# google-research/nerf-from-image

Hardware: NVIDIA H100
Metric: rays_per_sec_128x128_64+64spp (higher is better)
Workload: dtype f32

## Files before the change

nerf_from_image_b200/csrc/nfi_forward_pipe.cuh:

```cuda
#pragma once
#include <type_traits>

#include "nfi_forward.cuh"
#include "nfi_forward_tc.cuh"

namespace nfi {

#ifndef NFI_WAIT_NS
#define NFI_WAIT_NS 0
#endif
#define NFI_STEP_WAIT(bar, par) tc::mbar_wait_backoff<NFI_WAIT_NS>(bar, par)

__device__ __forceinline__ void mbar_arrive(uint64_t* bar) {
  asm volatile("mbarrier.arrive.shared::cta.b64 _, [%0];" ::"r"(tc::smem_u32(bar)) : "memory");
}

__device__ __forceinline__ float ld_relaxed(const float* p) {
  float v;
  asm volatile("ld.relaxed.cta.global.f32 %0, [%1];" : "=f"(v) : "l"(p) : "memory");
  return v;
}

__device__ __forceinline__ bool elect_one() {
  uint32_t pred;
  asm volatile(
      "{\n.reg .pred p;\nelect.sync _|p, 0xffffffff;\nselp.u32 %0, 1, 0, p;\n}\n"
      : "=r"(pred));
  return pred != 0;
}

struct TileCoord {
  int b, tile_x, tile_y;
};

__device__ __forceinline__ TileCoord tile_coord(int tile, int tiles_x, int tiles_y) {
  TileCoord c;
  const int per_img = tiles_x * tiles_y;
  c.b = tile / per_img;
  const int r = tile % per_img;
  const int bx = (tiles_x + 1) / 2;
  const int blk = r / 4, in = r % 4;
  int tx = 2 * (blk % bx) + (in & 1), ty = 2 * (blk / bx) + (in >> 1);
  if ((tiles_x & 1) || (tiles_y & 1)) {
    tx = r % tiles_x;
    ty = r / tiles_x;
  }
  c.tile_x = tx;
  c.tile_y = ty;
  return c;
}

constexpr int kPipeSlots = 3;
constexpr int kPipeStageBytes = 32768;
constexpr int kFwdStageBytes = 16384;
constexpr int kD2Ld = 20;
constexpr int kD2SlotBytes = kThreads * kD2Ld * 4;

__host__ __device__ inline size_t pipe_scratch_floats(int S, int nes) {
  return tc_scratch_floats_per_group(S) + (size_t)S * kThreads * nes;
}

constexpr int kViewTileBytes = kThreads * NFI_VIEW_FEATURES * 4;

template <int P, bool VD = false>
struct PipeCfg {
  static constexpr int kThreadsTotal = 256 + 128 * P;
  static constexpr int kStages = P + 1;
  static constexpr int kSmA = VD ? 41984 : 25600;
  static constexpr int kSmD2 = kSmA + kStages * kFwdStageBytes;
  static constexpr int kSmView = kSmD2 + kPipeSlots * kD2SlotBytes;
  static constexpr int kSmPal = kSmView + (VD ? kViewTileBytes : 0);
  static constexpr int kSmFrac = kSmPal + 48 * 4;
  static constexpr int kSmBars = kSmFrac + 128 * 4;
  static constexpr int kNumBars = 2 * kStages + 2 * kPipeSlots + 3;
  static constexpr int kSmBytes = kSmBars + kNumBars * 8;
  static constexpr int kActRegs = 136;
  static constexpr int kShadeRegs = 80;
  static constexpr int kProducerRegs = 88;
};

constexpr float kLog2e = 1.4426950408889634f;
constexpr float kLn2 = 0.6931471805599453f;
constexpr float kPadLogit = -1e30f;

__device__ __forceinline__ void decoder_layer2(const float (&d)[32], uint64_t w2_hi, uint64_t w2_lo,
                                               const float* __restrict__ b1, float* d2, int warp,
                                               int lane) {
  uint32_t hi[8][4], lo[8][4];
  tc::softplus_frag<true>(d, b1, lane & 3, hi, lo);
  float o[8];
#pragma unroll
  for (int i = 0; i < 8; ++i) o[i] = 0.f;
  tc::wgmma_fence();
  tc::layer2_mb(o, hi, lo, w2_hi, w2_lo);
  tc::wgmma_commit();
  tc::wgmma_wait<0>();
  tc::reg_fence(o);
  tc::store_frag_rows(o, d2, kD2Ld, warp, lane);
}

template <typename F>
__device__ __forceinline__ void decoder_step(uint64_t dsc_a, uint64_t w1_hi, uint64_t w1_lo,
                                             uint64_t w2_hi, uint64_t w2_lo,
                                             const float* __restrict__ b1, float* d2, int warp,
                                             int lane, F&& on_stage_read) {
#pragma unroll 1
  for (int mb = 0; mb < 2; ++mb) {
    float d[32];
#pragma unroll
    for (int i = 0; i < 32; ++i) d[i] = 0.f;
    tc::wgmma_fence();
    tc::layer1_mb(d, dsc_a + mb * (8192 >> 4), dsc_a + ((16384 + mb * 8192) >> 4), w1_hi, w1_lo);
    tc::wgmma_commit();
    tc::wgmma_wait<0>();
    tc::reg_fence(d);
    if (mb == 1) on_stage_read();
    decoder_layer2(d, w2_hi, w2_lo, b1, d2 + 64 * mb * kD2Ld, warp, lane);
  }
}

template <typename F>
__device__ __forceinline__ void decoder_step_fp32(const unsigned char* stage, uint64_t w1_hi,
                                                  uint64_t w1_lo, uint64_t w2_hi, uint64_t w2_lo,
                                                  const float* __restrict__ b1, float* d2, int warp,
                                                  int lane, F&& on_stage_read) {
  float fa[4][4], fb[4][4];
  tc::load_afrag_sw128(fa, stage, 0, warp, lane);
  tc::load_afrag_sw128(fb, stage, 64, warp, lane);
  on_stage_read();
#pragma unroll 1
  for (int mb = 0; mb < 2; ++mb) {
    uint32_t a_hi[4][4], a_lo[4][4];
#pragma unroll
    for (int kb = 0; kb < 4; ++kb)
#pragma unroll
      for (int s = 0; s < 4; ++s) tc::put_split(a_hi, a_lo, kb, s, fa[kb][s]);
    float d[32];
#pragma unroll
    for (int i = 0; i < 32; ++i) d[i] = 0.f;
    tc::wgmma_fence();
    tc::layer1_mb_rs(d, a_hi, a_lo, w1_hi, w1_lo);
    tc::wgmma_commit();
    tc::wgmma_wait<0>();
    tc::reg_fence(d);
    decoder_layer2(d, w2_hi, w2_lo, b1, d2 + 64 * mb * kD2Ld, warp, lane);
#pragma unroll
    for (int kb = 0; kb < 4; ++kb)
#pragma unroll
      for (int s = 0; s < 4; ++s) fa[kb][s] = fb[kb][s];
  }
}

__device__ __forceinline__ void fill_view_tile(const nfi_render_params& p, const TileCoord& tcd,
                                               const float* __restrict__ b2f, float4* vt, int wig,
                                               int lane) {
  const int g = lane >> 2, t = lane & 3;
#pragma unroll
  for (int mb = 0; mb < 2; ++mb) {
    const float* src[2];
#pragma unroll
    for (int h = 0; h < 2; ++h) {
      const int row = 64 * mb + 16 * wig + g + 8 * h;
      int px, py;
      tile_pixel(tcd.tile_x, tcd.tile_y, row >> 5, row & 31, px, py);
      px = min(px, p.width - 1);
      py = min(py, p.height - 1);
      const size_t ray = ((size_t)tcd.b * p.height + py) * p.width + px;
      src[h] = p.view_features + ray * NFI_VIEW_FEATURES + 2 * t;
    }
#pragma unroll
    for (int j = 0; j < NFI_VIEW_FEATURES / 8; ++j) {
      const float2 a = __ldg(reinterpret_cast<const float2*>(src[0] + 8 * j));
      const float2 c = __ldg(reinterpret_cast<const float2*>(src[1] + 8 * j));
      const float2 bb = *reinterpret_cast<const float2*>(b2f + 8 * j + 2 * t);
      vt[(mb * 4 + j) * kThreads] = make_float4(a.x + bb.x, a.y + bb.y, c.x + bb.x, c.y + bb.y);
    }
  }
}

__device__ __forceinline__ uint32_t decoder_layers23_vd(const float (&d)[32], uint64_t w2_hi,
                                                        uint64_t w2_lo, uint64_t w3_hi,
                                                        uint64_t w3_lo, const float* __restrict__ b1,
                                                        const float4* vt, float* d2, int warp,
                                                        int lane) {
  uint32_t hi[8][4], lo[8][4];
  tc::softplus_frag<true>(d, b1, lane & 3, hi, lo);
  float o[20];
#pragma unroll
  for (int i = 0; i < 20; ++i) o[i] = 0.f;
  tc::wgmma_fence();
  tc::layer2_vd_mb(o, hi, lo, w2_hi, w2_lo);
  tc::wgmma_commit();
  tc::wgmma_wait<0>();
  tc::reg_fence(o);
  uint32_t yhi[4][4], ylo[4][4];
  uint32_t neg = 0;
#pragma unroll
  for (int j = 0; j < 4; ++j) {
    const float4 v = vt[j * kThreads];
    const float ve[4] = {v.x, v.y, v.z, v.w};
#pragma unroll
    for (int e = 0; e < 4; ++e) {
      const float z = o[4 * j + e] + ve[e];
      tc::put_split(yhi, ylo, j, tc::afrag_slot(e), z > 0.f ? z : z * 0.2f);
      neg |= (z > 0.f ? 0u : 1u) << (4 * j + e);
    }
  }
  float q[8];
#pragma unroll
  for (int i = 0; i < 8; ++i) q[i] = 0.f;
  tc::wgmma_fence();
  tc::layer3_vd_mb(q, yhi, ylo, w3_hi, w3_lo);
  tc::wgmma_commit();
  tc::wgmma_wait<0>();
  tc::reg_fence(q);
  if ((lane & 3) == 0) {
    q[0] = o[16];
    q[2] = o[18];
  }
  tc::store_frag_rows(q, d2, kD2Ld, warp, lane);
  return neg;
}

template <typename F>
__device__ __forceinline__ uint32_t decoder_step_vd(const unsigned char* stage, uint64_t w1_hi,
                                                uint64_t w1_lo, uint64_t w2_hi, uint64_t w2_lo,
                                                uint64_t w3_hi, uint64_t w3_lo,
// ... 70 lines not shown
#pragma unroll
    for (int a = 0; a < NA; ++a) {
      const float e = tc::ex2_approx(out[1 + a] - m);
      if (probs != nullptr) probs[a] = e;
      s += e;
      r = fmaf(e, pv[3 * a + 0], r);
      g = fmaf(e, pv[3 * a + 1], g);
      b = fmaf(e, pv[3 * a + 2], b);
    }
    const float inv = __fdividef(1.f, s);
    cr = r * inv;
    cg = g * inv;
    cb = b * inv;
    if (probs != nullptr) {
#pragma unroll
      for (int a = 0; a < NA; ++a) probs[a] *= inv;
    }
  } else {
    cr = sigmoid_fast(out[1]) * 2.004f - 1.002f;
    cg = sigmoid_fast(out[2]) * 2.004f - 1.002f;
    cb = sigmoid_fast(out[3]) * 2.004f - 1.002f;
  }
}

template <int N>
struct LaneVec {
  float v[N];
};
template <int N>
__device__ __forceinline__ LaneVec<N> shift_down1(const LaneVec<N>& x, float pad, int lane) {
  LaneVec<N> y;
#pragma unroll
  for (int i = 0; i < N; ++i) {
    const float a = __shfl_down_sync(kFull, x.v[i], 1);
    const float nxt0 = (i + 1 < N) ? __shfl_sync(kFull, x.v[(i + 1 < N) ? i + 1 : i], 0) : pad;
    y.v[i] = (lane == 31) ? nxt0 : a;
  }
  return y;
}
template <int N>
__device__ __forceinline__ float pick(const LaneVec<N>& x, int idx) {
  float r = __shfl_sync(kFull, x.v[0], idx & 31);
#pragma unroll
  for (int i = 1; i < N; ++i) {
    const float t = __shfl_sync(kFull, x.v[i], idx & 31);
    r = ((idx >> 5) == i) ? t : r;
  }
  return r;
}
template <int N>
__device__ __forceinline__ void bitonic_sort(LaneVec<N>& x, int lane) {
#pragma unroll
  for (int k = 2; k <= 32 * N; k <<= 1) {
#pragma unroll
    for (int j = k >> 1; j > 0; j >>= 1) {
      if (j >= 32) {
        const int dj = j >> 5;
#pragma unroll
        for (int i = 0; i < N; ++i) {
          if ((i & dj) == 0) {
            const int ip = i | dj;
            const bool asc = (k >= 32 * N) ? true : (((32 * i) & k) == 0);
            const float lo = fminf(x.v[i], x.v[ip]), hi = fmaxf(x.v[i], x.v[ip]);
            x.v[i] = asc ? lo : hi;
            x.v[ip] = asc ? hi : lo;
          }
        }
      } else {
        const bool lower = (lane & j) == 0;
#pragma unroll
        for (int i = 0; i < N; ++i) {
          const float o = __shfl_xor_sync(kFull, x.v[i], j);
          const bool asc = (k >= 32 * N) ? true : (k < 32 ? ((lane & k) == 0) : (((32 * i) & k) == 0));
          x.v[i] = (lower == asc) ? fminf(x.v[i], o) : fmaxf(x.v[i], o);
        }
      }
    }
  }
}

template <int N>
__device__ __forceinline__ LaneVec<N> resample_ray(const LaneVec<N>& w, const LaneVec<N>& t,
                                                   LaneVec<N> u, bool sorted, int S, int lane) {
  const float inf = __int_as_float(0x7f800000);
  const LaneVec<N> w1 = shift_down1<N>(w, 0.f, lane);
  const LaneVec<N> w2 = shift_down1<N>(w1, 0.f, lane);
  LaneVec<N> q;
  float sum = 0.f;
#pragma unroll
  for (int i = 0; i < N; ++i) {
    float pm = ((fmaxf(w.v[i], w1.v[i]) + fmaxf(w1.v[i], w2.v[i])) * 0.5f + 0.01f) + 1e-5f;
    if (32 * i + lane >= S - 2) pm = 0.f;
    q.v[i] = pm;
    sum += pm;
  }
#pragma unroll
  for (int o = 16; o > 0; o >>= 1) sum += __shfl_xor_sync(kFull, sum, o);
#pragma unroll
  for (int i = 0; i < N; ++i) q.v[i] = q.v[i] / sum;
#pragma unroll
  for (int o = 1; o < 32; o <<= 1) {
#pragma unroll
    for (int i = 0; i < N; ++i) {
      const float y = __shfl_up_sync(kFull, q.v[i], o);
      if (lane >= o) q.v[i] += y;
    }
  }
#pragma unroll
  for (int i = 1; i < N; ++i) q.v[i] += __shfl_sync(kFull, q.v[i - 1], 31);
  LaneVec<N> c;
#pragma unroll
  for (int i = 0; i < N; ++i) {
    const float up = __shfl_up_sync(kFull, q.v[i], 1);
    const float prev31 = (i > 0) ? __shfl_sync(kFull, q.v[(i > 0) ? i - 1 : 0], 31) : 0.f;
    c.v[i] = (lane == 0) ? prev31 : up;
    if (32 * i + lane > S - 2) c.v[i] = inf;
  }
  const LaneVec<N> t1 = shift_down1<N>(t, 0.f, lane);
  LaneVec<N> bn;
#pragma unroll
  for (int i = 0; i < N; ++i) bn.v[i] = 0.5f * (t1.v[i] + t.v[i]);
  if (!sorted) bitonic_sort<N>(u, lane);
  LaneVec<N> z;
#pragma unroll
  for (int h = 0; h < N; ++h) {
    const float uu = u.v[h];
    int pos = 0;
#pragma unroll
    for (int s = 16 * N; s > 0; s >>= 1) {
      const float val = pick<N>(c, pos + s - 1);
      if (val <= uu) pos += s;
    }
    const int below = max(pos - 1, 0), above = min(pos, S - 2);
    const float c0 = pick<N>(c, below), c1 = pick<N>(c, above);
    const float b0 = pick<N>(bn, below), b1 = pick<N>(bn, above);
    float den = c1 - c0;
    if (den < 1e-5f) den = 1.f;
    z.v[h] = b0 + (uu - c0) / den * (b1 - b0);
  }
  return z;
}

struct ResampleArgs {
  const float* sc_w;
  float* sc_zf;
  float* z_fine;
  const float* noise_t;
  const float* noise_u;
  const float* frac;
  int S, wig;
  bool explicit_noise;
};
template <int N>
__device__ __forceinline__ void resample_rows_impl(const ResampleArgs& a, int first, int count,
                                                   float tnear, float tfar, size_t ray, bool valid,
                                                   int lane) {
  const int S = a.S;
  if (count <= 0) return;
  struct In {
    LaneVec<N> w, n, u;
    size_t rayj;
  };
  auto load = [&](int j, In& in) {
    in.rayj = ((size_t)__shfl_sync(kFull, (unsigned)(ray >> 32), j) << 32) |
              (size_t)__shfl_sync(kFull, (unsigned)ray, j);
    const int col = 32 * a.wig + j;
#pragma unroll
    for (int i = 0; i < N; ++i) {
      const int e = 32 * i + lane;
      in.w.v[i] = (e < S) ? ldcg(a.sc_w + e * kThreads + col) : 0.f;
      in.n.v[i] = 0.f;
      if (a.explicit_noise) {
        in.n.v[i] = (e < S) ? a.noise_t[in.rayj * S + e] : 0.f;
        in.u.v[i] = (e < S) ? a.noise_u[in.rayj * S + e] : 2.f;
      } else {
        in.u.v[i] = (e < S) ? linspace01(e, S) : 2.f;
      }
    }
  };
  In cur, nxt;
  load(first, cur);
#pragma unroll 1
  for (int j = first; j < first + count; ++j) {
    load(j + 1 < first + count ? j + 1 : j, nxt);
    const float nearj = __shfl_sync(kFull, tnear, j), farj = __shfl_sync(kFull, tfar, j);
    const bool validj = __shfl_sync(kFull, (int)valid, j) != 0;
    const int col = 32 * a.wig + j;
    const float spanj = farj - nearj;
    LaneVec<N> t;
#pragma unroll
    for (int i = 0; i < N; ++i)
      t.v[i] = lerp_torch(nearj, farj, a.frac[32 * i + lane]) + cur.n.v[i] * (spanj / (float)S);
    const LaneVec<N> z = resample_ray<N>(cur.w, t, cur.u, !a.explicit_noise, S, lane);
#pragma unroll
    for (int i = 0; i < N; ++i) {
      const int e = 32 * i + lane;
      if (e < S) a.sc_zf[e * kThreads + col] = z.v[i];
      if (a.z_fine != nullptr && validj && e < S) a.z_fine[cur.rayj * S + e] = z.v[i];
    }
    cur = nxt;
  }
}
template <int NOUT_PAD, int EXTRA, bool FINE, int P, bool DBG, int NSLOT = 2, bool VD = false>
__global__ void __launch_bounds__(PipeCfg<P>::kThreadsTotal, 1)
render_forward_pipe(const nfi_render_params p, const unsigned char* __restrict__ wimg,
                    float* __restrict__ scratch) {
  using Cfg = PipeCfg<P, VD>;
  static_assert(!(VD && DBG), "the phase timers are not instantiated for the view-conditioned kernel");
  constexpr int kImgBytes = VD ? kVdBytes : kWiBytes;
  constexpr int kImgB1 = VD ? kVdB1 : kWiB1, kImgB2 = VD ? kVdHead : kWiB2;
  constexpr int NA_ = NOUT_PAD - 1;
  constexpr int NE = (EXTRA == 1) ? 3 : (EXTRA == 2 ? NA_ : 0);
  constexpr int NES = (EXTRA == 2) ? NA_ : 0;
  extern __shared__ __align__(1024) unsigned char smem_raw[];
  unsigned char* base = smem_raw;
  const int tid = threadIdx.x, lane = tid & 31;
  const int hw_wg = __shfl_sync(kFull, tid >> 7, 0);
  const int wg = (hw_wg < P) ? hw_wg + 3 : (P + 1 - hw_wg);
  const int gt = tid & 127;
  const int wig = __shfl_sync(kFull, gt >> 5, 0);
  const int S = p.num_samples;

  uint64_t* bars = reinterpret_cast<uint64_t*>(base + Cfg::kSmBars);
  constexpr int NS = Cfg::kStages;
  uint64_t* full = bars;
  uint64_t* a_free = full + NS;
  uint64_t* d2_full = a_free + NS;
  uint64_t* slot_free = d2_full + kPipeSlots;
  uint64_t* cw_ready = slot_free + kPipeSlots;
  uint64_t* zf_ready = cw_ready + 1;
  uint64_t* wbar = zf_ready + 1;
  float* d2s = reinterpret_cast<float*>(base + Cfg::kSmD2);
  const float* b1s = reinterpret_cast<const float*>(base + kImgB1);
  const float* b2s = reinterpret_cast<const float*>(base + kImgB2);
  float* pal = reinterpret_cast<float*>(base + Cfg::kSmPal);
  float* frac = reinterpret_cast<float*>(base + Cfg::kSmFrac);
  if (tid < 128) frac[tid] = (float)tid / (float)S;

  if (tid == 0) {
    if (tc::smem_u32(base) & 1023u) __trap();
    for (int i = 0; i < NS; ++i) {
      tc::mbar_init(&full[i], kWarps);
      tc::mbar_init(&a_free[i], kWarps);
    }
    for (int i = 0; i < kPipeSlots; ++i) {
      tc::mbar_init(&d2_full[i], kWarps);
      tc::mbar_init(&slot_free[i], kWarps);
    }
    tc::mbar_init(cw_ready, kWarps);
    tc::mbar_init(zf_ready, (2 + P) * kWarps);
    tc::mbar_init(wbar, 1);
    tc::fence_mbar_init();
  }
  __syncthreads();
  if (tid == 0) {
    tc::mbar_expect_tx(wbar, kImgBytes);
    tc::tma_bulk_g2s(base, wimg, kImgBytes, wbar);
  }
  tc::mbar_wait(wbar, 0);

  const int tiles_x = (p.width + kTileW - 1) / kTileW;
  const int tiles_y = (p.height + kTileH - 1) / kTileH;
  const int n_tiles = tiles_x * tiles_y * p.batch;
  const int my_tiles =
      ((int)blockIdx.x < n_tiles) ? (n_tiles - 1 - (int)blockIdx.x) / (int)gridDim.x + 1 : 0;
  const uint32_t total_steps = (uint32_t)my_tiles * (uint32_t)S * (FINE ? 2u : 1u);
  const int R = p.plane_res;
  const float inv_range = 1.f / p.scene_range;
  const bool explicit_noise = (p.noise_mode == NFI_NOISE_EXPLICIT);
  const bool dbg_skip_gather = (p.mlp_mode & 0x100) != 0;
  const bool dbg_skip_consumer = (p.mlp_mode & 0x200) != 0;
  const bool dbg_window = (p.mlp_mode & 0x800) != 0;
  const bool dbg_time = DBG && (p.mlp_mode & 0x1000) && p.normals != nullptr && blockIdx.x == 0 &&
                        lane == 0 && (wg <= 3) && wg != 2 && wig == 0;
  long long tacc[DBG ? 10 : 1];
  long long tprev = 0;
  if (DBG)
    for (int i = 0; i < 10; ++i) tacc[i] = 0;
#define NFI_T(i)                         \
  if (DBG && dbg_time) {                 \
    const long long now__ = clock64();   \
    tacc[i] += now__ - tprev;            \
    tprev = now__;                       \
  }
  float* slab = scratch + (size_t)blockIdx.x * pipe_scratch_floats(S, NES);
  float4* sc_srgb = reinterpret_cast<float4*>(slab);
  float* sc_t = slab + (size_t)4 * S * kThreads;
  float* sc_w = sc_t + (size_t)S * kThreads;
  float* sc_zf = sc_w + (size_t)S * kThreads;
  float* sc_e = sc_zf + (size_t)S * kThreads;

  constexpr int kRsParts = 2 + P;
  auto rs_first = [](int part) {
    constexpr int base_rows = 32 / kRsParts, rem = 32 % kRsParts;
    return part * base_rows + min(max(part - 2, 0), rem);
  };
  auto resample_rows = [&](int part, float tnear, float tfar, size_t ray, bool valid) {
    const int first = rs_first(part), count = rs_first(part + 1) - first;
    ResampleArgs ra;
    ra.sc_w = sc_w;
    ra.sc_zf = sc_zf;
    ra.z_fine = p.z_fine;
    ra.noise_t = p.noise_t;
    ra.noise_u = p.noise_u;
    ra.frac = frac;
    ra.S = S;
    ra.wig = wig;
    ra.explicit_noise = explicit_noise;
    resample_rows_impl<NSLOT>(ra, first, count, tnear, tfar, ray, valid, lane);
  };

  if (wg >= 3) {
    asm volatile("setmaxnreg.dec.sync.aligned.u32 %0;" ::"n"(Cfg::kProducerRegs));
    const int set = wg - 3;
    uint32_t n = 0;
    uint32_t tile_it = 0;
    for (int tile = blockIdx.x; tile < n_tiles; tile += gridDim.x, ++tile_it) {
      const TileCoord tcd = tile_coord(tile, tiles_x, tiles_y);
      const int b = tcd.b;
      int px, py;
      tile_pixel(tcd.tile_x, tcd.tile_y, wig, lane, px, py);
      const bool valid = (px < p.width) && (py < p.height);
      px = min(px, p.width - 1);
      py = min(py, p.height - 1);
      const size_t ray = ((size_t)b * p.height + py) * p.width + px;
      Ray r;
      setup_ray(p, b, py, px, r);
      const float span = r.tfar - r.tnear;
      const uint32_t plane_bytes = (uint32_t)R * (uint32_t)R * 128u;
      const unsigned char* planes_b =
          reinterpret_cast<const unsigned char*>(p.planes) + (size_t)b * 3 * plane_bytes;
      for (int pass = 0; pass < (FINE ? 2 : 1); ++pass) {
        if (pass == 1) {
          tc::mbar_wait(cw_ready, tile_it & 1);
          resample_rows(2 + set, r.tnear, r.tfar, ray, valid);
          __threadfence_block();
          __syncwarp();
          if (lane == 0) mbar_arrive(zf_ready);
          tc::mbar_wait(zf_ready, tile_it & 1);
        }
        int s = (int)(((uint32_t)set + (uint32_t)P - (n % P)) % P);
        auto fetch = [&](int ss) -> float {
          if (ss >= S) return 0.f;
          if (pass == 0) return explicit_noise ? p.noise_t[ray * S + ss] : 0.f;
          return ld_relaxed(sc_zf + ss * kThreads + gt);
        };
        float nxt = fetch(s);
        for (; s < S; s += P) {
          const uint32_t st = (n + (uint32_t)s) % NS, u = (n + (uint32_t)s) / NS;
          unsigned char* const stage = base + Cfg::kSmA + st * kFwdStageBytes;
          const float cur = nxt;
          nxt = fetch(s + P);
          if (DBG && dbg_time) tprev = clock64();
          NFI_STEP_WAIT(&a_free[st], (u & 1) ^ 1);
          NFI_T(0)
          float t;
          if (pass == 0)
            t = lerp_torch(r.tnear, r.tfar, frac[s]) + cur * (span / (float)S);
          else
            t = cur;
          const float x0 = (r.ox + r.dx * t) * inv_range, x1 = (r.oy + r.dy * t) * inv_range,
                      x2 = (r.oz + r.dz * t) * inv_range;
          ByteTaps tp;
          byte_taps(x0, x1, R, 0u, tp.o[0], tp.fx[0], tp.fy[0]);
          byte_taps(x0, x2, R, plane_bytes >> 4, tp.o[1], tp.fx[1], tp.fy[1]);
          byte_taps(x1, x2, R, plane_bytes >> 3, tp.o[2], tp.fx[2], tp.fy[2]);
          NFI_T(1)
          if (dbg_window) {
            tp.o[0] &= 0x7FFu;
            tp.o[1] &= 0x7FFu;
            tp.o[2] &= 0x7FFu;
          }
          if (!dbg_skip_gather)
            gather_to_tiles_lean<TileStore::kFp32>(planes_b, R, tp, stage, nullptr, 32 * wig, lane);
          NFI_T(2)
          __syncwarp();
          if (lane == 0) mbar_arrive(&full[st]);
          NFI_T(3)
          if (DBG && dbg_time) tacc[9] += 1;
        }
        n += (uint32_t)S;
      }
    }
    if (DBG && dbg_time)
      for (int i = 0; i < 10; ++i) p.normals[i] = (float)tacc[i];
  } else if (wg == 0) {
    asm volatile("setmaxnreg.inc.sync.aligned.u32 %0;" ::"n"(Cfg::kActRegs));
    const uint32_t base_s = tc::smem_u32(base);
    const uint64_t dsc_w1_hi = tc::gmma_desc_sw128(base_s + kWiW1Hi);
    const uint64_t dsc_w1_lo = tc::gmma_desc_sw128(base_s + kWiW1Lo);
    const uint64_t dsc_w2_hi = tc::gmma_desc_sw128(base_s + (VD ? kVdW2Hi : kWiW2Hi));
    const uint64_t dsc_w2_lo = tc::gmma_desc_sw128(base_s + (VD ? kVdW2Lo : kWiW2Lo));
    const float4* vt = reinterpret_cast<const float4*>(base + Cfg::kSmView) + gt;
    uint32_t st = 0, u = 0, sl = 0, v = 0;
    auto activate = [&]() {
      if (DBG && dbg_time && tprev == 0) tprev = clock64();
      NFI_T(2)
      NFI_STEP_WAIT(&full[st], u & 1);
      NFI_STEP_WAIT(&slot_free[sl], (v & 1) ^ 1);
      NFI_T(0)
      float* d2 = d2s + sl * (kThreads * kD2Ld);
      if constexpr (VD) {
        decoder_step_vd(base + Cfg::kSmA + st * kFwdStageBytes, dsc_w1_hi, dsc_w1_lo, dsc_w2_hi,
                        dsc_w2_lo, tc::gmma_desc_sw128(base_s + kVdW3Hi),
                        tc::gmma_desc_sw128(base_s + kVdW3Lo), b1s, vt, d2, wig, lane, [&]() {
                          __syncwarp();
                          if (lane == 0) mbar_arrive(&a_free[st]);
                        });
      } else if (!dbg_skip_consumer) {
        decoder_step_fp32(base + Cfg::kSmA + st * kFwdStageBytes, dsc_w1_hi, dsc_w1_lo, dsc_w2_hi,
                          dsc_w2_lo, b1s, d2, wig, lane, [&]() {
                            __syncwarp();
                            if (lane == 0) mbar_arrive(&a_free[st]);
                          });
      } else {
        __syncwarp();
        if (lane == 0) mbar_arrive(&a_free[st]);
      }
      __syncwarp();
      if (lane == 0) mbar_arrive(&d2_full[sl]);
      if (++st == NS) { st = 0; ++u; }
      if (++sl == kPipeSlots) { sl = 0; ++v; }
      NFI_T(1)
      if (DBG && dbg_time) tacc[9] += 1;
    };
    uint32_t tile_it = 0;
    for (int tile = blockIdx.x; tile < n_tiles; tile += gridDim.x, ++tile_it) {
      if constexpr (VD)
        fill_view_tile(p, tile_coord(tile, tiles_x, tiles_y),
                       reinterpret_cast<const float*>(base + kVdB2f),
                       reinterpret_cast<float4*>(base + Cfg::kSmView) + gt, wig, lane);
      for (int s = 0; s < S; ++s) activate();
      if (FINE) {
        const TileCoord tcd = tile_coord(tile, tiles_x, tiles_y);
        int px, py;
        tile_pixel(tcd.tile_x, tcd.tile_y, wig, lane, px, py);
        const bool valid = (px < p.width) && (py < p.height);
        px = min(px, p.width - 1);
        py = min(py, p.height - 1);
        const size_t ray = ((size_t)tcd.b * p.height + py) * p.width + px;
        Ray r;
        setup_ray(p, tcd.b, py, px, r);
        tc::mbar_wait(cw_ready, tile_it & 1);
        NFI_T(3)
        resample_rows(1, r.tnear, r.tfar, ray, valid);
        __threadfence_block();
        __syncwarp();
        if (lane == 0) mbar_arrive(zf_ready);
        NFI_T(4)
        for (int s = 0; s < S; ++s) activate();
      }
    }
    if (DBG && dbg_time)
      for (int i = 0; i < 10; ++i) p.normals[16 + i] = (float)tacc[i];
  } else {
    asm volatile("setmaxnreg.dec.sync.aligned.u32 %0;" ::"n"(Cfg::kShadeRegs));
    uint32_t sl = 0, v = 0;
    FieldConst fc;
    fc.A = p.n_attention;
    fc.use_sdf = p.use_sdf;
    fc.inv_beta = p.use_sdf ? 1.f / p.beta[0] : 0.f;
    fc.inv_alpha = p.use_sdf ? 1.f / p.alpha[0] : 0.f;

    uint32_t tile_it = 0;
    for (int tile = blockIdx.x; tile < n_tiles; tile += gridDim.x, ++tile_it) {
      const TileCoord tcd = tile_coord(tile, tiles_x, tiles_y);
      const int b = tcd.b;
      int px, py;
      tile_pixel(tcd.tile_x, tcd.tile_y, wig, lane, px, py);
      const bool valid = (px < p.width) && (py < p.height);
      px = min(px, p.width - 1);
      py = min(py, p.height - 1);
      const size_t ray = ((size_t)b * p.height + py) * p.width + px;
      Ray r;
      setup_ray(p, b, py, px, r);
      const float span = r.tfar - r.tnear;

      tc::bar_sync(1, kThreads);
      if (gt < 48)
        pal[gt] = (p.n_attention > 0 && gt < p.n_attention * 3)
                      ? p.palette[(size_t)b * p.n_attention * 3 + gt]
                      : 0.f;
      tc::bar_sync(1, kThreads);
      Compositor<NE, true> comp;
      comp.init();

      auto shade = [&](float t, float& sigma, float& cr, float& cg, float& cb, float* ex) {
        const float* d2 = d2s + sl * (kThreads * kD2Ld) + gt * kD2Ld;
        if (DBG && dbg_time && tprev == 0) tprev = clock64();
        NFI_T(2)
        NFI_STEP_WAIT(&d2_full[sl], v & 1);
        NFI_T(0)
        float o16[16];
#pragma unroll
        for (int o4 = 0; o4 < 4; ++o4) {
          const float4 x = *reinterpret_cast<const float4*>(d2 + 4 * o4);
          o16[4 * o4] = x.x;
          o16[4 * o4 + 1] = x.y;
          o16[4 * o4 + 2] = x.z;
          o16[4 * o4 + 3] = x.w;
        }
        __syncwarp();
        if (lane == 0) mbar_arrive(&slot_free[sl]);
        if (++sl == kPipeSlots) { sl = 0; ++v; }
        const float wx = r.ox + r.dx * t, wy = r.oy + r.dy * t, wz = r.oz + r.dz * t;
        const float x0 = wx * inv_range, x1 = wy * inv_range, x2 = wz * inv_range;
        const float keep =
            (fabsf(x0) > 1.f || fabsf(x1) > 1.f || fabsf(x2) > 1.f) ? 0.f : 1.f;
        float out[NOUT_PAD];
#pragma unroll
        for (int o4 = 0; o4 < NOUT_PAD / 4; ++o4) {
          const float4 bb = *reinterpret_cast<const float4*>(b2s + 4 * o4);
          out[4 * o4] = o16[4 * o4] + bb.x;
          out[4 * o4 + 1] = o16[4 * o4 + 1] + bb.y;
          out[4 * o4 + 2] = o16[4 * o4 + 2] + bb.z;
          out[4 * o4 + 3] = o16[4 * o4 + 3] + bb.w;
        }
        if (dbg_skip_consumer) {
          sigma = out[0];
          cr = cg = cb = out[1];
        } else {
          field_head_fast<NOUT_PAD>(out, fc, pal, keep, sigma, cr, cg, cb,
                                    EXTRA == 2 ? ex : nullptr);
        }
        if (EXTRA == 1) {
          ex[0] = wx;
          ex[1] = wy;
          ex[2] = wz;
        }
        NFI_T(1)
        if (DBG && dbg_time) tacc[9] += 1;
      };

      {
        float wT = 1.f, prev_t = 0.f, prev_s = 0.f;
        const float4* nz4 = reinterpret_cast<const float4*>(p.noise_t + ray * S);
        const float4 zero4 = make_float4(0.f, 0.f, 0.f, 0.f);
        float4 nzc = explicit_noise ? nz4[0] : zero4;
        float4 nzn = (explicit_noise && S > 4) ? nz4[1] : zero4;
        const float jit = span / (float)S;
        for (int s = 0; s < S; ++s) {
          const int sq = s & 3;
          const float nz = sq == 0 ? nzc.x : (sq == 1 ? nzc.y : (sq == 2 ? nzc.z : nzc.w));
          const float t = lerp_torch(r.tnear, r.tfar, frac[s]) + nz * jit;
          if (sq == 3) {
            nzc = nzn;
            nzn = (explicit_noise && s + 5 < S) ? nz4[(s + 5) >> 2] : zero4;
          }
          float sigma, cr, cg, cb;
          float ex[NE > 0 ? NE : 1];
          shade(t, sigma, cr, cg, cb, ex);
          if (FINE) {
            sc_srgb[s * kThreads + gt] = make_float4(sigma, cr, cg, cb);
            sc_t[s * kThreads + gt] = t;
#pragma unroll
            for (int a = 0; a < NES; ++a) sc_e[((size_t)s * NES + a) * kThreads + gt] = ex[a];
            if (s > 0) {
              const float delta = (t - prev_t) * r.dn;
              const float a = 1.f - __expf(-prev_s * delta);
              sc_w[(s - 1) * kThreads + gt] = a * wT;
              wT = wT * ((1.f - a) + 1e-10f);
            }
            prev_t = t;
            prev_s = sigma;
          } else {
            comp.push(t, sigma, cr, cg, cb, ex, r.dn);
          }
          NFI_T(3)
        }
      }

      if (FINE) {
        sc_w[(S - 1) * kThreads + gt] = 0.f;
        __threadfence_block();
        __syncwarp();
        if (lane == 0) mbar_arrive(cw_ready);
        tc::mbar_wait(cw_ready, tile_it & 1);
        NFI_T(4)
        resample_rows(0, r.tnear, r.tfar, ray, valid);
        __threadfence_block();
        __syncwarp();
        if (lane == 0) mbar_arrive(zf_ready);
        tc::mbar_wait(zf_ready, tile_it & 1);
        NFI_T(5)

        int c = 0;
        float ct0 = ldcg(sc_t + gt), ct1 = ldcg(sc_t + kThreads + gt);
        float4 cq0 = __ldcg(sc_srgb + gt), cq1 = __ldcg(sc_srgb + kThreads + gt);
        auto take_coarse = [&]() {
          float ce[NE > 0 ? NE : 1];
          if (EXTRA == 1) {
            ce[0] = r.ox + r.dx * ct0;
            ce[1] = r.oy + r.dy * ct0;
            ce[2] = r.oz + r.dz * ct0;
          }
#pragma unroll
          for (int a = 0; a < NES; ++a) ce[a] = ldcg(sc_e + ((size_t)c * NES + a) * kThreads + gt);
          comp.push(ct0, cq0.x, cq0.y, cq0.z, cq0.w, ce, r.dn);
          ++c;
          ct0 = ct1;
          cq0 = cq1;
          if (c + 1 < S) {
            ct1 = ldcg(sc_t + (c + 1) * kThreads + gt);
            cq1 = __ldcg(sc_srgb + (c + 1) * kThreads + gt);
          }
        };
        float z0 = ldcg(sc_zf + gt);
        float z1 = (S > 1) ? ldcg(sc_zf + kThreads + gt) : 0.f;
        for (int k = 0; k < S; ++k) {
          const float z = z0;
          z0 = z1;
          z1 = (k + 2 < S) ? ldcg(sc_zf + (k + 2) * kThreads + gt) : 0.f;
          float sigma, cr, cg, cb;
          float ex[NE > 0 ? NE : 1];
          shade(z, sigma, cr, cg, cb, ex);
          while (c < S && ct0 <= z) take_coarse();
          comp.push(z, sigma, cr, cg, cb, ex, r.dn);
          NFI_T(3)
        }
        while (c < S) take_coarse();
        NFI_T(6)
      }

      if (valid) {
        float bg = 0.f;
        if (p.white_background) bg = 1.f - comp.am;
        p.rgb[ray * 3 + 0] = comp.ar + bg;
        p.rgb[ray * 3 + 1] = comp.ag + bg;
        p.rgb[ray * 3 + 2] = comp.ab + bg;
        p.depth[ray] = comp.ad;
        p.mask[ray] = comp.am;
        for (int q = 0; q < p.n_peers; ++q) {
          float* pr = p.peer_rgb[q] + ray * 3;
          pr[0] = comp.ar + bg;
          pr[1] = comp.ag + bg;
          pr[2] = comp.ab + bg;
          p.peer_depth[q][ray] = comp.ad;
          p.peer_mask[q][ray] = comp.am;
        }
        if (EXTRA == 1 && p.extra != nullptr)
          for (int a = 0; a < 3; ++a) p.extra[ray * 3 + a] = comp.ae[a];
        if (EXTRA == 2 && p.extra != nullptr)
          for (int a = 0; a < NE; ++a)
            if (a < p.n_attention) p.extra[ray * p.n_attention + a] = comp.ae[a];
      }
    }
    if (DBG && dbg_time)
      for (int i = 0; i < 10; ++i) p.normals[32 + i] = (float)tacc[i];
  }
#undef NFI_T
  __syncthreads();
  if (p.n_peers > 0 && p.peer_done != nullptr && tid == 0) {
    __threadfence_system();
    const unsigned done = atomicAdd(p.peer_done, 1u);
    if (done == gridDim.x - 1) {
      __threadfence();
      *p.peer_done = 0u;
      for (int q = 0; q < p.n_peers; ++q)
        asm volatile("st.release.sys.global.u32 [%0], %1;" ::"l"(p.peer_signal[q]), "r"(p.peer_epoch)
                     : "memory");
      const long long t0 = clock64();
      for (int q = 0; q < p.n_peers; ++q) {
        const uint32_t* flag = p.peer_signal_self + p.peer_rank[q];
        uint32_t v;
        do {
          asm volatile("ld.acquire.sys.global.u32 %0, [%1];" : "=r"(v) : "l"(flag) : "memory");
          if ((int)(v - p.peer_epoch) >= 0) break;
          __nanosleep(200);
          if (clock64() - t0 > 60000000000LL) __trap();
        } while (true);
      }
    }
  }
}

}
```

Before: 36.05 million.

## Interleave coarse pass of next tile with fine pass using double-buffered scratch

Reorders the per-block pass sequence so the coarse pass of tile i+1 runs before the fine pass of tile i, with scratch slabs, palettes and cw/zf barriers double-buffered by tile parity. In the non-VD fine kernel, resampling moves entirely to the producer warpgroups, which interleave resample rows opportunistically whenever the coarse weights are ready and the next stage is not yet free. This is meant to hide the resampling bubble and the full-CTA sync between coarse and fine passes. It costs twice the global scratch, extra barrier bookkeeping, and more complex control flow in the producers.

```diff
diff --git a/nerf_from_image_b200/csrc/nfi_forward_pipe.cuh b/nerf_from_image_b200/csrc/nfi_forward_pipe.cuh
--- a/nerf_from_image_b200/csrc/nfi_forward_pipe.cuh
+++ b/nerf_from_image_b200/csrc/nfi_forward_pipe.cuh
@@ -13,6 +13,17 @@
 
 __device__ __forceinline__ void mbar_arrive(uint64_t* bar) {
   asm volatile("mbarrier.arrive.shared::cta.b64 _, [%0];" ::"r"(tc::smem_u32(bar)) : "memory");
+}
+
+__device__ __forceinline__ bool mbar_test(uint64_t* bar, uint32_t parity) {
+  uint32_t ok;
+  asm volatile(
+      "{\n.reg .pred p;\nmbarrier.test_wait.parity.shared::cta.b64 p, [%1], %2;\n"
+      "selp.u32 %0, 1, 0, p;\n}\n"
+      : "=r"(ok)
+      : "r"(tc::smem_u32(bar)), "r"(parity)
+      : "memory");
+  return ok != 0;
 }
 
 __device__ __forceinline__ float ld_relaxed(const float* p) {
@@ -56,8 +67,11 @@
 constexpr int kD2Ld = 20;
 constexpr int kD2SlotBytes = kThreads * kD2Ld * 4;
 
+__host__ __device__ inline size_t pipe_tile_scratch_floats(int S, int nes) {
+  return tc_scratch_floats_per_group(S) + (size_t)S * kThreads * nes;
+}
 __host__ __device__ inline size_t pipe_scratch_floats(int S, int nes) {
-  return tc_scratch_floats_per_group(S) + (size_t)S * kThreads * nes;
+  return 2 * pipe_tile_scratch_floats(S, nes);
 }
 
 constexpr int kViewTileBytes = kThreads * NFI_VIEW_FEATURES * 4;
@@ -70,9 +84,9 @@
   static constexpr int kSmD2 = kSmA + kStages * kFwdStageBytes;
   static constexpr int kSmView = kSmD2 + kPipeSlots * kD2SlotBytes;
   static constexpr int kSmPal = kSmView + (VD ? kViewTileBytes : 0);
-  static constexpr int kSmFrac = kSmPal + 48 * 4;
+  static constexpr int kSmFrac = kSmPal + 2 * 48 * 4;
   static constexpr int kSmBars = kSmFrac + 128 * 4;
-  static constexpr int kNumBars = 2 * kStages + 2 * kPipeSlots + 3;
+  static constexpr int kNumBars = 2 * kStages + 2 * kPipeSlots + 5;
   static constexpr int kSmBytes = kSmBars + kNumBars * 8;
   static constexpr int kActRegs = 136;
   static constexpr int kShadeRegs = 80;
@@ -449,54 +463,76 @@
   bool explicit_noise;
 };
 template <int N>
+struct ResampleIn {
+  LaneVec<N> w, n, u;
+  size_t rayj;
+};
+template <int N>
+__device__ __forceinline__ void resample_load(const ResampleArgs& a, int j, size_t ray, int lane,
+                                              ResampleIn<N>& in) {
+  const int S = a.S;
+  in.rayj = ((size_t)__shfl_sync(kFull, (unsigned)(ray >> 32), j) << 32) |
+            (size_t)__shfl_sync(kFull, (unsigned)ray, j);
+  const int col = 32 * a.wig + j;
+#pragma unroll
+  for (int i = 0; i < N; ++i) {
+    const int e = 32 * i + lane;
+    in.w.v[i] = (e < S) ? ldcg(a.sc_w + e * kThreads + col) : 0.f;
+    in.n.v[i] = 0.f;
+    if (a.explicit_noise) {
+      in.n.v[i] = (e < S) ? a.noise_t[in.rayj * S + e] : 0.f;
+      in.u.v[i] = (e < S) ? a.noise_u[in.rayj * S + e] : 2.f;
+    } else {
+      in.u.v[i] = (e < S) ? linspace01(e, S) : 2.f;
+    }
+  }
+}
+template <int N>
+__device__ __forceinline__ void resample_store(const ResampleArgs& a, int j, const ResampleIn<N>& in,
+                                               float tnear, float tfar, bool valid, int lane) {
+  const int S = a.S;
+  const float nearj = __shfl_sync(kFull, tnear, j), farj = __shfl_sync(kFull, tfar, j);
+  const bool validj = __shfl_sync(kFull, (int)valid, j) != 0;
+  const int col = 32 * a.wig + j;
+  const float spanj = farj - nearj;
+  LaneVec<N> t;
+#pragma unroll
+  for (int i = 0; i < N; ++i)
+    t.v[i] = lerp_torch(nearj, farj, a.frac[32 * i + lane]) + in.n.v[i] * (spanj / (float)S);
+  const LaneVec<N> z = resample_ray<N>(in.w, t, in.u, !a.explicit_noise, S, lane);
+#pragma unroll
+  for (int i = 0; i < N; ++i) {
+    const int e = 32 * i + lane;
+    if (e < S) a.sc_zf[e * kThreads + col] = z.v[i];
+    if (a.z_fine != nullptr && validj && e < S) a.z_fine[in.rayj * S + e] = z.v[i];
+  }
+}
+template <int N>
 __device__ __forceinline__ void resample_rows_impl(const ResampleArgs& a, int first, int count,
                                                    float tnear, float tfar, size_t ray, bool valid,
                                                    int lane) {
-  const int S = a.S;
   if (count <= 0) return;
-  struct In {
-    LaneVec<N> w, n, u;
-    size_t rayj;
-  };
-  auto load = [&](int j, In& in) {
-    in.rayj = ((size_t)__shfl_sync(kFull, (unsigned)(ray >> 32), j) << 32) |
-              (size_t)__shfl_sync(kFull, (unsigned)ray, j);
-    const int col = 32 * a.wig + j;
-#pragma unroll
-    for (int i = 0; i < N; ++i) {
-      const int e = 32 * i + lane;
-      in.w.v[i] = (e < S) ? ldcg(a.sc_w + e * kThreads + col) : 0.f;
-      in.n.v[i] = 0.f;
-      if (a.explicit_noise) {
-        in.n.v[i] = (e < S) ? a.noise_t[in.rayj * S + e] : 0.f;
-        in.u.v[i] = (e < S) ? a.noise_u[in.rayj * S + e] : 2.f;
-      } else {
-        in.u.v[i] = (e < S) ? linspace01(e, S) : 2.f;
-      }
-    }
-  };
-  In cur, nxt;
-  load(first, cur);
+  ResampleIn<N> cur, nxt;
+  resample_load<N>(a, first, ray, lane, cur);
 #pragma unroll 1
   for (int j = first; j < first + count; ++j) {
-    load(j + 1 < first + count ? j + 1 : j, nxt);
-    const float nearj = __shfl_sync(kFull, tnear, j), farj = __shfl_sync(kFull, tfar, j);
-    const bool validj = __shfl_sync(kFull, (int)valid, j) != 0;
-    const int col = 32 * a.wig + j;
-    const float spanj = farj - nearj;
-    LaneVec<N> t;
-#pragma unroll
-    for (int i = 0; i < N; ++i)
-      t.v[i] = lerp_torch(nearj, farj, a.frac[32 * i + lane]) + cur.n.v[i] * (spanj / (float)S);
-    const LaneVec<N> z = resample_ray<N>(cur.w, t, cur.u, !a.explicit_noise, S, lane);
-#pragma unroll
-    for (int i = 0; i < N; ++i) {
-      const int e = 32 * i + lane;
-      if (e < S) a.sc_zf[e * kThreads + col] = z.v[i];
-      if (a.z_fine != nullptr && validj && e < S) a.z_fine[cur.rayj * S + e] = z.v[i];
-    }
+    resample_load<N>(a, j + 1 < first + count ? j + 1 : j, ray, lane, nxt);
+    resample_store<N>(a, j, cur, tnear, tfar, valid, lane);
     cur = nxt;
   }
+}
+
+struct PipePass {
+  int i;
+  bool fine;
+};
+template <bool FINE, bool AHEAD>
+__device__ __forceinline__ PipePass pipe_pass(int q, int T) {
+  if (!FINE) return {q, false};
+  if (!AHEAD) return {q >> 1, (q & 1) != 0};
+  if (q == 0) return {0, false};
+  if (q == 2 * T - 1) return {T - 1, true};
+  return (q & 1) ? PipePass{(q + 1) >> 1, false} : PipePass{(q >> 1) - 1, true};
 }
 template <int NOUT_PAD, int EXTRA, bool FINE, int P, bool DBG, int NSLOT = 2, bool VD = false>
 __global__ void __launch_bounds__(PipeCfg<P>::kThreadsTotal, 1)
@@ -520,17 +556,19 @@
 
   uint64_t* bars = reinterpret_cast<uint64_t*>(base + Cfg::kSmBars);
   constexpr int NS = Cfg::kStages;
+  constexpr bool kAhead = FINE && !VD;
+  constexpr int kRsParts = kAhead ? P : 2 + P;
   uint64_t* full = bars;
   uint64_t* a_free = full + NS;
   uint64_t* d2_full = a_free + NS;
   uint64_t* slot_free = d2_full + kPipeSlots;
   uint64_t* cw_ready = slot_free + kPipeSlots;
-  uint64_t* zf_ready = cw_ready + 1;
-  uint64_t* wbar = zf_ready + 1;
+  uint64_t* zf_ready = cw_ready + 2;
+  uint64_t* wbar = zf_ready + 2;
   float* d2s = reinterpret_cast<float*>(base + Cfg::kSmD2);
   const float* b1s = reinterpret_cast<const float*>(base + kImgB1);
   const float* b2s = reinterpret_cast<const float*>(base + kImgB2);
-  float* pal = reinterpret_cast<float*>(base + Cfg::kSmPal);
+  float* pals = reinterpret_cast<float*>(base + Cfg::kSmPal);
   float* frac = reinterpret_cast<float*>(base + Cfg::kSmFrac);
   if (tid < 128) frac[tid] = (float)tid / (float)S;
 
@@ -544,8 +582,10 @@
       tc::mbar_init(&d2_full[i], kWarps);
       tc::mbar_init(&slot_free[i], kWarps);
     }
-    tc::mbar_init(cw_ready, kWarps);
-    tc::mbar_init(zf_ready, (2 + P) * kWarps);
+    for (int i = 0; i < 2; ++i) {
+      tc::mbar_init(&cw_ready[i], kWarps);
+      tc::mbar_init(&zf_ready[i], kRsParts * kWarps);
+    }
     tc::mbar_init(wbar, 1);
     tc::fence_mbar_init();
   }
@@ -561,7 +601,7 @@
   const int n_tiles = tiles_x * tiles_y * p.batch;
   const int my_tiles =
       ((int)blockIdx.x < n_tiles) ? (n_tiles - 1 - (int)blockIdx.x) / (int)gridDim.x + 1 : 0;
-  const uint32_t total_steps = (uint32_t)my_tiles * (uint32_t)S * (FINE ? 2u : 1u);
+  const int n_pass = my_tiles * (FINE ? 2 : 1);
   const int R = p.plane_res;
   const float inv_range = 1.f / p.scene_range;
   const bool explicit_noise = (p.noise_mode == NFI_NOISE_EXPLICIT);
@@ -580,23 +620,32 @@
     tacc[i] += now__ - tprev;            \
     tprev = now__;                       \
   }
-  float* slab = scratch + (size_t)blockIdx.x * pipe_scratch_floats(S, NES);
-  float4* sc_srgb = reinterpret_cast<float4*>(slab);
-  float* sc_t = slab + (size_t)4 * S * kThreads;
-  float* sc_w = sc_t + (size_t)S * kThreads;
-  float* sc_zf = sc_w + (size_t)S * kThreads;
-  float* sc_e = sc_zf + (size_t)S * kThreads;
-
-  constexpr int kRsParts = 2 + P;
+  float* const slabs = scratch + (size_t)blockIdx.x * pipe_scratch_floats(S, NES);
+  auto slab_of = [&](int i) { return slabs + (size_t)(i & 1) * pipe_tile_scratch_floats(S, NES); };
+  auto sc_w_of = [&](int i) { return slab_of(i) + (size_t)5 * S * kThreads; };
+  auto sc_zf_of = [&](int i) { return slab_of(i) + (size_t)6 * S * kThreads; };
+
+  auto row_ray = [&](int i, int& b, size_t& ray, bool& valid, Ray& r) {
+    const TileCoord tcd = tile_coord((int)blockIdx.x + i * (int)gridDim.x, tiles_x, tiles_y);
+    b = tcd.b;
+    int px, py;
+    tile_pixel(tcd.tile_x, tcd.tile_y, wig, lane, px, py);
+    valid = (px < p.width) && (py < p.height);
+    px = min(px, p.width - 1);
+    py = min(py, p.height - 1);
+    ray = ((size_t)b * p.height + py) * p.width + px;
+    setup_ray(p, b, py, px, r);
+  };
+
   auto rs_first = [](int part) {
     constexpr int base_rows = 32 / kRsParts, rem = 32 % kRsParts;
-    return part * base_rows + min(max(part - 2, 0), rem);
+    return kAhead ? part * base_rows + min(part, rem)
+                  : part * base_rows + min(max(part - 2, 0), rem);
   };
-  auto resample_rows = [&](int part, float tnear, float tfar, size_t ray, bool valid) {
-    const int first = rs_first(part), count = rs_first(part + 1) - first;
+  auto resample_args = [&](int i) {
     ResampleArgs ra;
-    ra.sc_w = sc_w;
-    ra.sc_zf = sc_zf;
+    ra.sc_w = sc_w_of(i);
+    ra.sc_zf = sc_zf_of(i);
     ra.z_fine = p.z_fine;
     ra.noise_t = p.noise_t;
     ra.noise_u = p.noise_u;
@@ -604,80 +653,120 @@
     ra.S = S;
     ra.wig = wig;
     ra.explicit_noise = explicit_noise;
-    resample_rows_impl<NSLOT>(ra, first, count, tnear, tfar, ray, valid, lane);
+    return ra;
+  };
+  auto resample_rows = [&](int i, int part, float tnear, float tfar, size_t ray, bool valid) {
+    const int first = rs_first(part), count = rs_first(part + 1) - first;
+    resample_rows_impl<NSLOT>(resample_args(i), first, count, tnear, tfar, ray, valid, lane);
   };
 
   if (wg >= 3) {
     asm volatile("setmaxnreg.dec.sync.aligned.u32 %0;" ::"n"(Cfg::kProducerRegs));
     const int set = wg - 3;
+    const int rs_part = kAhead ? set : 2 + set;
     uint32_t n = 0;
-    uint32_t tile_it = 0;
-    for (int tile = blockIdx.x; tile < n_tiles; tile += gridDim.x, ++tile_it) {
-      const TileCoord tcd = tile_coord(tile, tiles_x, tiles_y);
-      const int b = tcd.b;
-      int px, py;
-      tile_pixel(tcd.tile_x, tcd.tile_y, wig, lane, px, py);
-      const bool valid = (px < p.width) && (py < p.height);
-      px = min(px, p.width - 1);
-      py = min(py, p.height - 1);
-      const size_t ray = ((size_t)b * p.height + py) * p.width + px;
+    int rs_i = -1, rs_j = 0, rs_end = 0;
+    float rs_tnear = 0.f, rs_tfar = 0.f;
+    size_t rs_ray = 0;
+    bool rs_valid = false;
+    auto rows_begin = [&](int i) {
+      int bb;
+      Ray rr;
+      row_ray(i, bb, rs_ray, rs_valid, rr);
+      rs_tnear = rr.tnear;
+      rs_tfar = rr.tfar;
+      rs_i = i;
+      rs_j = rs_first(rs_part);
+      rs_end = rs_first(rs_part + 1);
+    };
+    auto row_next = [&]() {
+      const ResampleArgs ra = resample_args(rs_i);
+      ResampleIn<NSLOT> in;
+      resample_load<NSLOT>(ra, rs_j, rs_ray, lane, in);
+      resample_store<NSLOT>(ra, rs_j, in, rs_tnear, rs_tfar, rs_valid, lane);
+      ++rs_j;
+    };
+    for (int q = 0; q < n_pass; ++q) {
+      const PipePass ps = pipe_pass<FINE, kAhead>(q, my_tiles);
+      int b;
+      size_t ray;
+      bool valid;
       Ray r;
-      setup_ray(p, b, py, px, r);
+      row_ray(ps.i, b, ray, valid, r);
       const float span = r.tfar - r.tnear;
       const uint32_t plane_bytes = (uint32_t)R * (uint32_t)R * 128u;
       const unsigned char* planes_b =
           reinterpret_cast<const unsigned char*>(p.planes) + (size_t)b * 3 * plane_bytes;
-      for (int pass = 0; pass < (FINE ? 2 : 1); ++pass) {
-        if (pass == 1) {
-          tc::mbar_wait(cw_ready, tile_it & 1);
-          resample_rows(2 + set, r.tnear, r.tfar, ray, valid);
-          __threadfence_block();
-          __syncwarp();
-          if (lane == 0) mbar_arrive(zf_ready);
-          tc::mbar_wait(zf_ready, tile_it & 1);
-        }
-        int s = (int)(((uint32_t)set + (uint32_t)P - (n % P)) % P);
-        auto fetch = [&](int ss) -> float {
-          if (ss >= S) return 0.f;
-          if (pass == 0) return explicit_noise ? p.noise_t[ray * S + ss] : 0.f;
-          return ld_relaxed(sc_zf + ss * kThreads + gt);
-        };
-        float nxt = fetch(s);
-        for (; s < S; s += P) {
-          const uint32_t st = (n + (uint32_t)s) % NS, u = (n + (uint32_t)s) / NS;
-          unsigned char* const stage = base + Cfg::kSmA + st * kFwdStageBytes;
-          const float cur = nxt;
-          nxt = fetch(s + P);
-          if (DBG && dbg_time) tprev = clock64();
-          NFI_STEP_WAIT(&a_free[st], (u & 1) ^ 1);
-          NFI_T(0)
-          float t;
-          if (pass == 0)
-            t = lerp_torch(r.tnear, r.tfar, frac[s]) + cur * (span / (float)S);
-          else
-            t = cur;
-          const float x0 = (r.ox + r.dx * t) * inv_range, x1 = (r.oy + r.dy * t) * inv_range,
-                      x2 = (r.oz + r.dz * t) * inv_range;
-          ByteTaps tp;
-          byte_taps(x0, x1, R, 0u, tp.o[0], tp.fx[0], tp.fy[0]);
-          byte_taps(x0, x2, R, plane_bytes >> 4, tp.o[1], tp.fx[1], tp.fy[1]);
-          byte_taps(x1, x2, R, plane_bytes >> 3, tp.o[2], tp.fx[2], tp.fy[2]);
-          NFI_T(1)
-          if (dbg_window) {
-            tp.o[0] &= 0x7FFu;
-            tp.o[1] &= 0x7FFu;
-            tp.o[2] &= 0x7FFu;
-          }
-          if (!dbg_skip_gather)
-            gather_to_tiles_lean<TileStore::kFp32>(planes_b, R, tp, stage, nullptr, 32 * wig, lane);
-          NFI_T(2)
-          __syncwarp();
-          if (lane == 0) mbar_arrive(&full[st]);
-          NFI_T(3)
-          if (DBG && dbg_time) tacc[9] += 1;
-        }
-        n += (uint32_t)S;
-      }
+      const float* const sc_zf = sc_zf_of(ps.i);
+      uint64_t* const zf = zf_ready + (ps.i & 1);
+      const uint32_t tpar = ((uint32_t)ps.i >> 1) & 1u;
+      if (ps.fine) {
+        if (kAhead) {
+          if (rs_i != ps.i) rows_begin(ps.i);
+          tc::mbar_wait(cw_ready + (ps.i & 1), tpar);
+          while (rs_j < rs_end) row_next();
+        } else {
+          tc::mbar_wait(cw_ready + (ps.i & 1), tpar);
+          resample_rows(ps.i, rs_part, r.tnear, r.tfar, ray, valid);
+        }
+        __threadfence_block();
+        __syncwarp();
+        if (lane == 0) mbar_arrive(zf);
+        tc::mbar_wait(zf, tpar);
+      } else if (kAhead && ps.i > 0) {
+        rows_begin(ps.i - 1);
+      }
+      int s = (int)(((uint32_t)set + (uint32_t)P - (n % P)) % P);
+      auto fetch = [&](int ss) -> float {
+        if (ss >= S) return 0.f;
+        if (!ps.fine) return explicit_noise ? p.noise_t[ray * S + ss] : 0.f;
+        return ld_relaxed(sc_zf + ss * kThreads + gt);
+      };
+      float nxt = fetch(s);
+      for (; s < S; s += P) {
+        const uint32_t st = (n + (uint32_t)s) % NS, u = (n + (uint32_t)s) / NS;
+        unsigned char* const stage = base + Cfg::kSmA + st * kFwdStageBytes;
+        const float cur = nxt;
+        nxt = fetch(s + P);
+        if (DBG && dbg_time) tprev = clock64();
+        while (kAhead && rs_j < rs_end) {
+          uint64_t* const cw = cw_ready + (rs_i & 1);
+          const uint32_t cpar = ((uint32_t)rs_i >> 1) & 1u;
+          if (!__shfl_sync(kFull, (int)(mbar_test(cw, cpar) && !mbar_test(&a_free[st], (u & 1) ^ 1)),
+                           0))
+            break;
+          tc::mbar_wait(cw, cpar);
+          row_next();
+          NFI_T(4)
+        }
+        NFI_STEP_WAIT(&a_free[st], (u & 1) ^ 1);
+        NFI_T(0)
+        float t;
+        if (!ps.fine)
+          t = lerp_torch(r.tnear, r.tfar, frac[s]) + cur * (span / (float)S);
+        else
+          t = cur;
+        const float x0 = (r.ox + r.dx * t) * inv_range, x1 = (r.oy + r.dy * t) * inv_range,
+                    x2 = (r.oz + r.dz * t) * inv_range;
+        ByteTaps tp;
+        byte_taps(x0, x1, R, 0u, tp.o[0], tp.fx[0], tp.fy[0]);
+        byte_taps(x0, x2, R, plane_bytes >> 4, tp.o[1], tp.fx[1], tp.fy[1]);
+        byte_taps(x1, x2, R, plane_bytes >> 3, tp.o[2], tp.fx[2], tp.fy[2]);
+        NFI_T(1)
+        if (dbg_window) {
+          tp.o[0] &= 0x7FFu;
+          tp.o[1] &= 0x7FFu;
+          tp.o[2] &= 0x7FFu;
+        }
+        if (!dbg_skip_gather)
+          gather_to_tiles_lean<TileStore::kFp32>(planes_b, R, tp, stage, nullptr, 32 * wig, lane);
+        NFI_T(2)
+        __syncwarp();
+        if (lane == 0) mbar_arrive(&full[st]);
+        NFI_T(3)
+        if (DBG && dbg_time) tacc[9] += 1;
+      }
+      n += (uint32_t)S;
     }
     if (DBG && dbg_time)
       for (int i = 0; i < 10; ++i) p.normals[i] = (float)tacc[i];
@@ -690,12 +779,16 @@
     const uint64_t dsc_w2_lo = tc::gmma_desc_sw128(base_s + (VD ? kVdW2Lo : kWiW2Lo));
     const float4* vt = reinterpret_cast<const float4*>(base + Cfg::kSmView) + gt;
     uint32_t st = 0, u = 0, sl = 0, v = 0;
-    auto activate = [&]() {
+    auto activate = [&](bool fine0) {
       if (DBG && dbg_time && tprev == 0) tprev = clock64();
       NFI_T(2)
       NFI_STEP_WAIT(&full[st], u & 1);
       NFI_STEP_WAIT(&slot_free[sl], (v & 1) ^ 1);
-      NFI_T(0)
+      if (fine0) {
+        NFI_T(5)
+      } else {
+        NFI_T(0)
+      }
       float* d2 = d2s + sl * (kThreads * kD2Ld);
       if constexpr (VD) {
         decoder_step_vd(base + Cfg::kSmA + st * kFwdStageBytes, dsc_w1_hi, dsc_w1_lo, dsc_w2_hi,
@@ -721,32 +814,28 @@
       NFI_T(1)
       if (DBG && dbg_time) tacc[9] += 1;
     };
-    uint32_t tile_it = 0;
-    for (int tile = blockIdx.x; tile < n_tiles; tile += gridDim.x, ++tile_it) {
+    for (int q = 0; q < n_pass; ++q) {
+      const PipePass ps = pipe_pass<FINE, kAhead>(q, my_tiles);
       if constexpr (VD)
-        fill_view_tile(p, tile_coord(tile, tiles_x, tiles_y),
-                       reinterpret_cast<const float*>(base + kVdB2f),
-                       reinterpret_cast<float4*>(base + Cfg::kSmView) + gt, wig, lane);
-      for (int s = 0; s < S; ++s) activate();
-      if (FINE) {
-        const TileCoord tcd = tile_coord(tile, tiles_x, tiles_y);
-        int px, py;
-        tile_pixel(tcd.tile_x, tcd.tile_y, wig, lane, px, py);
-        const bool valid = (px < p.width) && (py < p.height);
-        px = min(px, p.width - 1);
-        py = min(py, p.height - 1);
-        const size_t ray = ((size_t)tcd.b * p.height + py) * p.width + px;
+        if (!ps.fine)
+          fill_view_tile(p, tile_coord((int)blockIdx.x + ps.i * (int)gridDim.x, tiles_x, tiles_y),
+                         reinterpret_cast<const float*>(base + kVdB2f),
+                         reinterpret_cast<float4*>(base + Cfg::kSmView) + gt, wig, lane);
+      if (!kAhead && ps.fine) {
+        int b;
+        size_t ray;
+        bool valid;
         Ray r;
-        setup_ray(p, tcd.b, py, px, r);
-        tc::mbar_wait(cw_ready, tile_it & 1);
+        row_ray(ps.i, b, ray, valid, r);
+        tc::mbar_wait(cw_ready + (ps.i & 1), ((uint32_t)ps.i >> 1) & 1u);
         NFI_T(3)
-        resample_rows(1, r.tnear, r.tfar, ray, valid);
+        resample_rows(ps.i, 1, r.tnear, r.tfar, ray, valid);
         __threadfence_block();
         __syncwarp();
-        if (lane == 0) mbar_arrive(zf_ready);
+        if (lane == 0) mbar_arrive(zf_ready + (ps.i & 1));
         NFI_T(4)
-        for (int s = 0; s < S; ++s) activate();
-      }
+      }
+      for (int s = 0; s < S; ++s) activate(ps.fine && s == 0);
     }
     if (DBG && dbg_time)
       for (int i = 0; i < 10; ++i) p.normals[16 + i] = (float)tacc[i];
@@ -759,26 +848,31 @@
     fc.inv_beta = p.use_sdf ? 1.f / p.beta[0] : 0.f;
     fc.inv_alpha = p.use_sdf ? 1.f / p.alpha[0] : 0.f;
 
-    uint32_t tile_it = 0;
-    for (int tile = blockIdx.x; tile < n_tiles; tile += gridDim.x, ++tile_it) {
-      const TileCoord tcd = tile_coord(tile, tiles_x, tiles_y);
-      const int b = tcd.b;
-      int px, py;
-      tile_pixel(tcd.tile_x, tcd.tile_y, wig, lane, px, py);
-      const bool valid = (px < p.width) && (py < p.height);
-      px = min(px, p.width - 1);
-      py = min(py, p.height - 1);
-      const size_t ray = ((size_t)b * p.height + py) * p.width + px;
+    for (int q = 0; q < n_pass; ++q) {
+      const PipePass ps = pipe_pass<FINE, kAhead>(q, my_tiles);
+      int b;
+      size_t ray;
+      bool valid;
       Ray r;
-      setup_ray(p, b, py, px, r);
+      row_ray(ps.i, b, ray, valid, r);
       const float span = r.tfar - r.tnear;
-
-      tc::bar_sync(1, kThreads);
-      if (gt < 48)
-        pal[gt] = (p.n_attention > 0 && gt < p.n_attention * 3)
-                      ? p.palette[(size_t)b * p.n_attention * 3 + gt]
-                      : 0.f;
-      tc::bar_sync(1, kThreads);
+      float* const slab = slab_of(ps.i);
+      float4* const sc_srgb = reinterpret_cast<float4*>(slab);
+      float* const sc_t = slab + (size_t)4 * S * kThreads;
+      float* const sc_w = sc_w_of(ps.i);
+      float* const sc_zf = sc_zf_of(ps.i);
+      float* const sc_e = sc_zf + (size_t)S * kThreads;
+      float* const pal = pals + 48 * (ps.i & 1);
+      const uint32_t tpar = ((uint32_t)ps.i >> 1) & 1u;
+
+      if (!ps.fine) {
+        tc::bar_sync(1, kThreads);
+        if (gt < 48)
+          pal[gt] = (p.n_attention > 0 && gt < p.n_attention * 3)
+                        ? p.palette[(size_t)b * p.n_attention * 3 + gt]
+                        : 0.f;
+        tc::bar_sync(1, kThreads);
+      }
       Compositor<NE, true> comp;
       comp.init();
 
@@ -829,7 +923,7 @@
         if (DBG && dbg_time) tacc[9] += 1;
       };
 
-      {
+      if (!ps.fine) {
         float wT = 1.f, prev_t = 0.f, prev_s = 0.f;
         const float4* nz4 = reinterpret_cast<const float4*>(p.noise_t + ray * S);
         const float4 zero4 = make_float4(0.f, 0.f, 0.f, 0.f);
@@ -848,14 +942,14 @@
           float ex[NE > 0 ? NE : 1];
           shade(t, sigma, cr, cg, cb, ex);
           if (FINE) {
-            sc_srgb[s * kThreads + gt] = make_float4(sigma, cr, cg, cb);
-            sc_t[s * kThreads + gt] = t;
-#pragma unroll
-            for (int a = 0; a < NES; ++a) sc_e[((size_t)s * NES + a) * kThreads + gt] = ex[a];
+            reinterpret_cast<float4*>(slab)[s * kThreads + gt] = make_float4(sigma, cr, cg, cb);
+            slab[(4 * S + s) * kThreads + gt] = t;
+#pragma unroll
+            for (int a = 0; a < NES; ++a) slab[(7 * S + s * NES + a) * kThreads + gt] = ex[a];
             if (s > 0) {
               const float delta = (t - prev_t) * r.dn;
               const float a = 1.f - __expf(-prev_s * delta);
-              sc_w[(s - 1) * kThreads + gt] = a * wT;
+              slab[(5 * S + s - 1) * kThreads + gt] = a * wT;
               wT = wT * ((1.f - a) + 1e-10f);
             }
             prev_t = t;
@@ -867,18 +961,24 @@
         }
       }
 
-      if (FINE) {
+      if (FINE && !ps.fine) {
         sc_w[(S - 1) * kThreads + gt] = 0.f;
         __threadfence_block();
         __syncwarp();
-        if (lane == 0) mbar_arrive(cw_ready);
-        tc::mbar_wait(cw_ready, tile_it & 1);
+        if (lane == 0) mbar_arrive(cw_ready + (ps.i & 1));
+        if (!kAhead) {
+          tc::mbar_wait(cw_ready + (ps.i & 1), tpar);
+          resample_rows(ps.i, 0, r.tnear, r.tfar, ray, valid);
+          __threadfence_block();
+          __syncwarp();
+          if (lane == 0) mbar_arrive(zf_ready + (ps.i & 1));
+        }
         NFI_T(4)
-        resample_rows(0, r.tnear, r.tfar, ray, valid);
-        __threadfence_block();
-        __syncwarp();
-        if (lane == 0) mbar_arrive(zf_ready);
-        tc::mbar_wait(zf_ready, tile_it & 1);
+        continue;
+      }
+
+      if (FINE) {
+        tc::mbar_wait(zf_ready + (ps.i & 1), tpar);
         NFI_T(5)
 
         int c = 0;
```

After: 37.15 million, median of 6. +3.0%, better.
